# ChainSafe/Spectre

Hardware: NVIDIA H100
Metric: bn254_g1_msm_pairs_per_s (higher is better)
Workload: dtype u256 (8x32-bit Montgomery limbs, INT32 IMAD)

## Files before the change

### spectre_b200/csrc/common.cuh

```cuda
#pragma once
#include <cuda_runtime.h>
#include <stdint.h>
#include <stdio.h>
#include <string.h>
#include <initializer_list>
#include <map>
#include <mutex>
#include <string>
#include <vector>
#include "curve.cuh"
#include "../../include/spectre_b200.h"

namespace spb {


struct DevBuf {
  void* ptr = nullptr;
  size_t cap = 0;
};

struct NttTables {
  Fr omega;
  uint32_t k, h;
  Fr* tw_lo = nullptr;
  Fr* tw_hi = nullptr;
  Fr* tw_full = nullptr;
};

struct MsmLane {
  cudaStream_t stream = nullptr;
  cudaEvent_t ev[9] = {nullptr, nullptr, nullptr, nullptr, nullptr, nullptr, nullptr, nullptr, nullptr};
  void* pinned = nullptr;
  bool ready = false;
};
static const int kMaxMsmLanes = 3;

struct DeviceState {
  int device = 0;
  int sm_count = 0;
  size_t total_mem = 0;
  cudaStream_t stream = nullptr;
  cudaEvent_t ev0 = nullptr, ev1 = nullptr;
  cudaEvent_t dep_ev = nullptr;
  cudaEvent_t stage_ev[8] = {nullptr, nullptr, nullptr, nullptr, nullptr, nullptr, nullptr, nullptr};
  std::map<std::string, DevBuf> slots;
  MsmLane lanes[kMaxMsmLanes];
  std::vector<NttTables> ntt_tables;
  std::vector<NttTables> ntt_pre_tables;
  void* pinned = nullptr;
  size_t pinned_cap = 0;
  void* stage[2] = {nullptr, nullptr};
  cudaEvent_t stage_done[2] = {nullptr, nullptr};
};

}

struct spb_ctx {
  std::vector<spb::DeviceState> dev;
  std::mutex mu;
  std::string last_error;
  bool peer_access = false;
  uint64_t n_kernel_launches = 0;
  float last_kernel_ms = 0.f;
  uint64_t last_msm_adds = 0;
  bool shplonk_slots_busy = false;
  float msm_stage_ms[7] = {0, 0, 0, 0, 0, 0, 0};
};

struct spb_domain {
  uint32_t j, k, extended_k, quotient_poly_degree;
  spb::Fr omega, omega_inv, extended_omega, extended_omega_inv, g_coset, g_coset_inv, ifft_divisor, extended_ifft_divisor;
  uint32_t t_len;
  spb::Fr* d_t_evaluations;
  int device;
};

namespace spb {

int set_error(spb_ctx* ctx, int code, const char* fmt, ...);
void* slot(spb_ctx* ctx, DeviceState& d, const char* name, size_t bytes);

#define SPB_CUDA(ctx, call)                                                                      \
  do {                                                                                           \
    cudaError_t e_ = (call);                                                                     \
// ... 122 lines not shown
```

### spectre_b200/csrc/msm.cu

```cuda
#define SPB_MSM_KERNELS 1
#include "common.cuh"
#include "msm.cuh"
#include <cub/device/device_scan.cuh>
#include <string.h>

using namespace spb;

struct SrsShard {
  int dev_index = 0;
  size_t start = 0, count = 0;
  G1Affine* g = nullptr;
  G1Affine* g_lagrange = nullptr;
};
struct spb_srs {
  uint32_t k = 0;
  size_t n = 0;
  unsigned char g2[128] = {0}, s_g2[128] = {0};
  uint32_t table_c = 0;
  std::vector<SrsShard> shards;
};


namespace spb {

typedef MsmLane Lane;
static const size_t kLanePinnedBytes = 256 * 1024;
static int get_lane(spb_ctx* ctx, int dev_index, int lane_index, Lane** out) {
  Lane& l = ctx->dev[dev_index].lanes[lane_index];
  if (!l.ready) {
    SPB_CUDA(ctx, cudaStreamCreateWithFlags(&l.stream, cudaStreamNonBlocking));
    for (int i = 0; i < 9; i++) SPB_CUDA(ctx, cudaEventCreate(&l.ev[i]));
    SPB_CUDA(ctx, cudaMallocHost(&l.pinned, kLanePinnedBytes));
    l.ready = true;
  }
  *out = &l;
  return 0;
}

void msm_release_ctx(spb_ctx* ctx) {
  for (auto& d : ctx->dev) {
    cudaSetDevice(d.device);
    for (auto& l : d.lanes) {
      if (!l.ready) continue;
      cudaStreamSynchronize(l.stream);
      for (int i = 0; i < 9; i++) cudaEventDestroy(l.ev[i]);
      cudaFreeHost(l.pinned);
      cudaStreamDestroy(l.stream);
      l = Lane();
    }
  }
}

static void* lane_slot(spb_ctx* ctx, DeviceState& d, int lane, const char* name, size_t bytes) {
  char buf[64];
  snprintf(buf, sizeof buf, "%s#%d", name, lane);
  return slot(ctx, d, buf, bytes);
}

static uint32_t choose_chunk(const DeviceState& d, uint64_t est_entries) {
  const double wave = (double)d.sm_count * 512.0;
  if (est_entries >= kLongChunkMinEntries) return kLongChunk;
  double waves = (double)est_entries / 32.0 / wave;
  if (waves < 1.0) return 32;
  double w = waves < 1.5 ? 1.0 : (double)(uint64_t)(waves + 0.5);
  uint32_t L = (uint32_t)((double)est_entries / (w * wave)) + 1;
  if (L < 24) L = 24;
  if (L > 48) L = 48;
  return L;
}

static int msm_enqueue(spb_ctx* ctx, DeviceState& d, int lane, Lane& ln, const Fr* d_scalars, const G1Affine* d_bases, uint64_t n, MsmGeom g) {
  const uint64_t nb = (uint64_t)g.BW * g.B;
  const uint64_t cap = n * g.W;
  const uint32_t Lmin = g.L == kLongChunk ? kShortChunk : g.L;
  const uint64_t Tmax = (cap + Lmin - 1) / Lmin;
  if (cap >= 0x7fffffffull) return set_error(ctx, SPB_ERR_ARG, "msm: %llu entries exceed the 31-bit sort index", (unsigned long long)cap);
  uint32_t* counts = (uint32_t*)lane_slot(ctx, d, lane, "msm_counts", (nb + 1) * 4);
  uint32_t* offsets = (uint32_t*)lane_slot(ctx, d, lane, "msm_offsets", (nb + 1) * 4);
  MsmEntry* ent = (MsmEntry*)lane_slot(ctx, d, lane, "msm_entries", (cap + 1) * sizeof(MsmEntry));
  G1Xyzz* buckets = (G1Xyzz*)lane_slot(ctx, d, lane, "msm_buckets", nb * sizeof(G1Xyzz));
  uint32_t* head_key = (uint32_t*)lane_slot(ctx, d, lane, "msm_head_key", (Tmax + 1) * 4);
  uint32_t* tail_key = (uint32_t*)lane_slot(ctx, d, lane, "msm_tail_key", (Tmax + 1) * 4);
  G1Xyzz* head = (G1Xyzz*)lane_slot(ctx, d, lane, "msm_head", (Tmax + 1) * sizeof(G1Xyzz));
  G1Xyzz* tail = (G1Xyzz*)lane_slot(ctx, d, lane, "msm_tail", (Tmax + 1) * sizeof(G1Xyzz));
  uint32_t* giant = (uint32_t*)lane_slot(ctx, d, lane, "msm_giant", (Tmax + 2) * 4);
  const uint64_t max_huge = Tmax / kHugeChain + 1;
  uint32_t* huge = (uint32_t*)lane_slot(ctx, d, lane, "msm_huge", (2 * max_huge + 2) * 4);
  G1Xyzz* huge_part = (G1Xyzz*)lane_slot(ctx, d, lane, "msm_huge_part", max_huge * kHugeBlocks * sizeof(G1Xyzz));
  const MsmTail tl = msm_tail_shape(g.c);
  const uint32_t R = 1u << tl.r_log, C = 1u << tl.c_log, per = msm_tail_partials(tl);
  const uint32_t T1 = g.B >> tl.m_log;
  const uint64_t ngroups = (uint64_t)g.BW * T1;
  G1Xyzz* grp = (G1Xyzz*)lane_slot(ctx, d, lane, "msm_groups", 2 * ngroups * sizeof(G1Xyzz));
  G1Xyzz* seg_out = (G1Xyzz*)lane_slot(ctx, d, lane, "msm_rowcol", (uint64_t)g.BW * (2 * R + C) * sizeof(G1Xyzz));
  G1Xyzz* win_out = (G1Xyzz*)lane_slot(ctx, d, lane, "msm_partials", (uint64_t)g.BW * per * sizeof(G1Xyzz));
  size_t scan_bytes = 0;
  cub::DeviceScan::ExclusiveSum(nullptr, scan_bytes, counts, offsets, (int)(nb + 1), ln.stream);
  void* scan_tmp = lane_slot(ctx, d, lane, "msm_scan_tmp", scan_bytes ? scan_bytes : 16);
  if (!counts || !offsets || !ent || !buckets || !head_key || !tail_key || !head || !tail || !giant || !huge || !huge_part || !grp || !seg_out || !win_out || !scan_tmp)
    return SPB_ERR_OOM;
  if ((size_t)g.BW * per * sizeof(G1Xyzz) + 16 > kLanePinnedBytes) return set_error(ctx, SPB_ERR_STATE, "msm: %u window partials exceed the pinned staging area", g.BW * per);

  cudaStream_t st = ln.stream;
  SPB_CUDA(ctx, cudaMemsetAsync(giant, 0, 4, st));
  SPB_CUDA(ctx, cudaMemsetAsync(huge, 0, 4, st));
  const unsigned tb = 256;
  SPB_CUDA(ctx, cudaMemsetAsync(counts, 0, (nb + 1) * 4, st));
  cudaEventRecord(ln.ev[0], st);
  SPB_TRY(launch(ctx, st, nblk(n, tb), tb, 0, msm_count_kernel, n, d_scalars, g, counts));
  cudaEventRecord(ln.ev[1], st);
  SPB_CUDA(ctx, cub::DeviceScan::ExclusiveSum(scan_tmp, scan_bytes, counts, offsets, (int)(nb + 1), st));
  SPB_CUDA(ctx, cudaMemcpyAsync(counts, offsets, (nb + 1) * 4, cudaMemcpyDeviceToDevice, st));
  cudaEventRecord(ln.ev[2], st);
  SPB_TRY(launch(ctx, st, nblk(n, tb), tb, 0, msm_scatter_kernel, n, d_scalars, g, counts, ent));
  const uint32_t* total = offsets + nb;
  cudaEventRecord(ln.ev[3], st);
  SPB_TRY(launch(ctx, st, nblk(Tmax, 128), 128, 0, msm_accumulate_kernel, total, g, ent, d_bases, buckets, head_key, head, tail_key, tail));
  cudaEventRecord(ln.ev[4], st);
  SPB_TRY(launch(ctx, st, nblk(Tmax, 128), 128, 0, msm_stitch_kernel, total, g.L, 24, head_key, head, tail_key, tail, buckets, giant, giant + 1));
  SPB_TRY(launch(ctx, st, 256, 128, 0, msm_giant_kernel, total, g.L, giant, giant + 1, head_key, head, tail_key, tail, buckets, huge, huge + 2));
  SPB_TRY(launch(ctx, st, kHugeBlocks, 128, 0, msm_huge_kernel, huge, huge + 2, head, huge_part));
  SPB_TRY(launch(ctx, st, 64, 128, 0, msm_huge_finish_kernel, huge, huge + 2, kHugeBlocks, huge_part, tail_key, tail, buckets));
  cudaEventRecord(ln.ev[5], st);
  G1Xyzz *rows = seg_out, *cols = seg_out + (uint64_t)g.BW * R, *wrows = seg_out + (uint64_t)g.BW * (R + C);
  SPB_TRY(launch(ctx, st, nblk(ngroups, 128), 128, 0, msm_group_kernel, ngroups, tl.m_log, offsets, buckets, grp, grp + ngroups));
  cudaEventRecord(ln.ev[6], st);
  SPB_TRY(launch(ctx, st, g.BW * (2 * R + C), 64, 0, msm_rowcol_kernel, T1, tl, grp, grp + ngroups, rows, cols, wrows));
  SPB_TRY(launch(ctx, st, g.BW * (2 * tl.nbr + tl.nbc), 128, 0, msm_weighted_kernel, tl, rows, cols, wrows, win_out));
  cudaEventRecord(ln.ev[7], st);
  SPB_CUDA(ctx, cudaMemcpyAsync(ln.pinned, win_out, (size_t)g.BW * per * sizeof(G1Xyzz), cudaMemcpyDeviceToHost, st));
  SPB_CUDA(ctx, cudaMemcpyAsync((char*)ln.pinned + (size_t)g.BW * per * sizeof(G1Xyzz), total, 4, cudaMemcpyDeviceToHost, st));
  return 0;
}

static G1Xyzz msm_finish(Lane& ln, MsmGeom g, uint64_t* adds) {
  const MsmTail tl = msm_tail_shape(g.c);
  const uint32_t per = msm_tail_partials(tl);
  const G1Xyzz* P = (const G1Xyzz*)ln.pinned;
  uint32_t M; memcpy(&M, (const char*)ln.pinned + (size_t)g.BW * per * sizeof(G1Xyzz), 4);
  if (adds) *adds += (uint64_t)M + 2ull * g.BW * g.B;
  std::vector<G1Xyzz> S(g.BW);
  for (uint32_t w = 0; w < g.BW; w++) S[w] = msm_tail_finish(g, P + (size_t)w * per);
  return msm_combine_windows(S.data(), g.BW, g.c);
}

static void write_result(const G1Xyzz& r, spb_g1* out) {
  G1Affine a = xyzz_to_affine(r);
  G1Jac j = jac_from_affine(a);
  memcpy(out, &j, sizeof(G1Jac));
}

struct MsmPart {
  int dev_index;
  const Fr* d_scalars;
  const Fr* h_scalars;
  int peer_src_device;
  const G1Affine* d_bases;
  uint64_t n;
  MsmGeom g;
};

static int job_enqueue(spb_ctx* ctx, int lane, std::vector<MsmPart>& parts) {
  for (auto& p : parts) {
    if (!p.n) continue;
    DeviceState& d = ctx->dev[p.dev_index];
    SPB_CUDA(ctx, cudaSetDevice(d.device));
    Lane* ln; SPB_TRY(get_lane(ctx, p.dev_index, lane, &ln));
    p.g.L = choose_chunk(d, p.n * p.g.W);
    const Fr* ds = p.d_scalars;
    DeviceState& src = p.peer_src_device >= 0 ? ctx->dev[0] : d;
    if (&src != &d) SPB_CUDA(ctx, cudaSetDevice(src.device));
    SPB_CUDA(ctx, cudaEventRecord(src.dep_ev, src.stream));
    if (&src != &d) SPB_CUDA(ctx, cudaSetDevice(d.device));
    SPB_CUDA(ctx, cudaStreamWaitEvent(ln->stream, src.dep_ev, 0));
    SPB_CUDA(ctx, cudaEventRecord(ln->ev[8], ln->stream));
    if (p.h_scalars || p.peer_src_device >= 0) {
      Fr* buf = (Fr*)lane_slot(ctx, d, lane, "msm_scalars", p.n * sizeof(Fr));
      if (!buf) return SPB_ERR_OOM;
      if (p.h_scalars) SPB_CUDA(ctx, cudaMemcpyAsync(buf, p.h_scalars, p.n * sizeof(Fr), cudaMemcpyHostToDevice, ln->stream));
      else SPB_CUDA(ctx, cudaMemcpyPeerAsync(buf, d.device, p.d_scalars, p.peer_src_device, p.n * sizeof(Fr), ln->stream));
      ds = buf;
    }
    SPB_TRY(msm_enqueue(ctx, d, lane, *ln, ds, p.d_bases, p.n, p.g));
  }
  return 0;
}

static int job_collect(spb_ctx* ctx, int lane, const std::vector<MsmPart>& parts, spb_g1* out) {
  G1Xyzz acc = xyzz_identity();
  float worst = 0.f;
  for (auto& p : parts) {
    if (!p.n) continue;
    DeviceState& d = ctx->dev[p.dev_index];
    SPB_CUDA(ctx, cudaSetDevice(d.device));
    Lane* ln; SPB_TRY(get_lane(ctx, p.dev_index, lane, &ln));
    SPB_CUDA(ctx, cudaStreamSynchronize(ln->stream));
    float ms = 0.f;
    SPB_CUDA(ctx, cudaEventElapsedTime(&ms, ln->ev[8], ln->ev[7]));
    if (ms > worst) worst = ms;
    if (p.dev_index == 0) for (int e = 0; e < 7; e++) cudaEventElapsedTime(&ctx->msm_stage_ms[e], ln->ev[e], ln->ev[e + 1]);
    G1Xyzz r = msm_finish(*ln, p.g, &ctx->last_msm_adds);
    xyzz_add(acc, r);
  }
  ctx->last_kernel_ms = worst;
  write_result(acc, out);
  return 0;
}

static int g1_fixed_base_mul(spb_ctx* ctx, DeviceState& d, const Fr* scalars, size_t n, G1Affine* out) {
  return launch(ctx, d.stream, nblk(n, 128), 128, 0, g1_fixed_base_mul_kernel, scalars, n, out);
}

}

extern "C" {

uint64_t spb_last_msm_adds(spb_ctx* ctx) { return ctx ? ctx->last_msm_adds : 0; }
void spb_last_msm_stage_ms(spb_ctx* ctx, float out[7]) { if (!out) return; for (int i = 0; i < 7; i++) out[i] = ctx ? ctx->msm_stage_ms[i] : 0.f; }
void spb_msm_geometry(size_t n, int tables, uint32_t* c, uint32_t* windows) {
  MsmGeom g = msm_make_geometry(msm_choose_c(n ? n : 1, tables != 0), tables != 0, 0);
  if (c) *c = g.c;
  if (windows) *windows = g.W;
}

static spb_srs* srs_alloc(spb_ctx* ctx, uint32_t k) {
  spb_srs* s = new spb_srs();
  s->k = k; s->n = (size_t)1 << k;
  size_t D = ctx->dev.size();
  for (size_t i = 0; i < D; i++) {
    SrsShard sh; sh.dev_index = (int)i;
    sh.start = s->n * i / D; sh.count = s->n * (i + 1) / D - sh.start;
    s->shards.push_back(sh);
  }
  return s;
}

// ... 298 lines not shown
    if (!src) return set_error(ctx, SPB_ERR_STATE, "spb_srs_download: basis %d not resident", basis);
    DeviceState& d = ctx->dev[sh.dev_index];
    SPB_CUDA(ctx, cudaSetDevice(d.device));
    SPB_CUDA(ctx, cudaMemcpy((G1Affine*)out + (lo - start), src + (lo - sh.start), (hi - lo) * sizeof(G1Affine), cudaMemcpyDeviceToHost));
  }
  return 0;
}

int spb_msm_raw(spb_ctx* ctx, const spb_fr* scalars, const spb_g1_affine* bases, size_t n, spb_g1* out) {
  if (!ctx || !out || (n && (!scalars || !bases))) return SPB_ERR_ARG;
  std::lock_guard<std::mutex> lk(ctx->mu);
  ctx->last_msm_adds = 0;
  std::vector<MsmPart> parts;
  size_t D = ctx->dev.size();
  for (size_t i = 0; i < D; i++) {
    size_t lo = n * i / D, cnt = n * (i + 1) / D - lo;
    if (!cnt) continue;
    DeviceState& d = ctx->dev[i];
    SPB_CUDA(ctx, cudaSetDevice(d.device));
    Lane* ln; SPB_TRY(get_lane(ctx, (int)i, 0, &ln));
    G1Affine* db = (G1Affine*)slot(ctx, d, "msm_raw_bases", cnt * sizeof(G1Affine));
    if (!db) return SPB_ERR_OOM;
    SPB_CUDA(ctx, cudaMemcpyAsync(db, (const G1Affine*)bases + lo, cnt * sizeof(G1Affine), cudaMemcpyHostToDevice, ln->stream));
    MsmPart p; p.dev_index = (int)i; p.d_scalars = nullptr; p.h_scalars = (const Fr*)scalars + lo; p.peer_src_device = -1;
    p.d_bases = db; p.n = cnt; p.g = msm_choose_geometry(cnt);
    parts.push_back(p);
  }
  SPB_TRY(job_enqueue(ctx, 0, parts));
  return job_collect(ctx, 0, parts, out);
}

static int srs_parts(spb_ctx* ctx, const spb_srs* srs, int basis, const Fr* scalars, bool on_device, size_t n, std::vector<MsmPart>& parts) {
  if (n > srs->n) return set_error(ctx, SPB_ERR_ARG, "spb_msm: %zu scalars but the SRS has %zu points", n, srs->n);
  for (auto& sh : srs->shards) {
    if (sh.start >= n) continue;
    size_t cnt = (n - sh.start) < sh.count ? (n - sh.start) : sh.count;
    const G1Affine* b = basis == SPB_BASIS_G ? sh.g : sh.g_lagrange;
    if (!b) return set_error(ctx, SPB_ERR_STATE, "spb_msm: basis %d not resident", basis);
    MsmPart p; p.dev_index = sh.dev_index; p.d_bases = b; p.n = cnt; p.h_scalars = nullptr; p.d_scalars = nullptr; p.peer_src_device = -1;
    if (!on_device) p.h_scalars = scalars + sh.start;
    else { p.d_scalars = scalars + sh.start; if (sh.dev_index != 0) p.peer_src_device = ctx->dev[0].device; }
    p.g = srs->table_c ? msm_make_geometry(srs->table_c, true, (uint32_t)sh.count) : msm_choose_geometry(cnt);
    parts.push_back(p);
  }
  return 0;
}

static int msm_batch_common(spb_ctx* ctx, const spb_srs* srs, int basis, const spb_fr* const* scalars, bool on_device, size_t n, size_t count, spb_g1* out) {
  if (!ctx || !srs || !out || (count && !scalars)) return SPB_ERR_ARG;
  std::lock_guard<std::mutex> lk(ctx->mu);
  ctx->last_msm_adds = 0;
  const MsmGeom lg = srs->table_c ? msm_make_geometry(srs->table_c, true, 0) : msm_choose_geometry(n ? n : 1);
  const uint64_t ents = (uint64_t)n * lg.W;
  const uint64_t lane_bytes = ents * sizeof(MsmEntry) + 2 * (ents / kShortChunk + 1) * (sizeof(G1Xyzz) + 4) + (uint64_t)lg.BW * lg.B * sizeof(G1Xyzz);
  const uint64_t fit = ctx->dev[0].total_mem / 10 / (lane_bytes ? lane_bytes : 1);
  const size_t NL = std::max<size_t>(1, std::min<size_t>((size_t)kMaxMsmLanes, (size_t)fit));
  std::vector<MsmPart> jobs[kMaxMsmLanes];
  for (size_t i = 0; i < count; i++) {
    int lane = (int)(i % NL);
    if (i >= NL) SPB_TRY(job_collect(ctx, lane, jobs[lane], &out[i - NL]));
    if (n && !scalars[i]) return SPB_ERR_ARG;
    jobs[lane].clear();
    SPB_TRY(srs_parts(ctx, srs, basis, (const Fr*)scalars[i], on_device, n, jobs[lane]));
    SPB_TRY(job_enqueue(ctx, lane, jobs[lane]));
  }
  for (size_t i = count >= NL ? count - NL : 0; i < count; i++) SPB_TRY(job_collect(ctx, (int)(i % NL), jobs[i % NL], &out[i]));
  return 0;
}

int spb_msm(spb_ctx* ctx, const spb_srs* srs, int basis, const spb_fr* scalars, size_t n, spb_g1* out) {
  const spb_fr* one[1] = {scalars};
  if (n && !scalars) return SPB_ERR_ARG;
  return msm_batch_common(ctx, srs, basis, one, false, n, 1, out);
}
int spb_msm_dev(spb_ctx* ctx, const spb_srs* srs, int basis, const spb_fr* d_scalars, size_t n, spb_g1* out) {
  const spb_fr* one[1] = {d_scalars};
  if (n && !d_scalars) return SPB_ERR_ARG;
  return msm_batch_common(ctx, srs, basis, one, true, n, 1, out);
}
int spb_msm_batch(spb_ctx* ctx, const spb_srs* srs, int basis, const spb_fr* const* scalars, size_t n, size_t count, spb_g1* out) {
  return msm_batch_common(ctx, srs, basis, scalars, false, n, count, out);
}
int spb_msm_batch_dev(spb_ctx* ctx, const spb_srs* srs, int basis, const spb_fr* const* d_scalars, size_t n, size_t count, spb_g1* out) {
  return msm_batch_common(ctx, srs, basis, d_scalars, true, n, count, out);
}

int spb_srs_precompute(spb_ctx* ctx, spb_srs* srs) {
  if (!ctx || !srs) return SPB_ERR_ARG;
  std::lock_guard<std::mutex> lk(ctx->mu);
  if (srs->table_c) return 0;
  size_t per_dev = srs->shards.empty() ? srs->n : srs->shards[0].count;
  uint32_t c = msm_choose_c(per_dev ? per_dev : 1, true);
  uint32_t W = (255 + c - 1) / c;
  for (auto& sh : srs->shards) {
    if (!sh.count) continue;
    SPB_CUDA(ctx, cudaSetDevice(ctx->dev[sh.dev_index].device));
    size_t free_b = 0, total_b = 0;
    SPB_CUDA(ctx, cudaMemGetInfo(&free_b, &total_b));
    const size_t bases = (sh.g ? 1 : 0) + (sh.g_lagrange ? 1 : 0);
    if ((size_t)W * sh.count * sizeof(G1Affine) * bases > total_b / 4) return 0;
  }
  for (auto& sh : srs->shards) {
    if (!sh.count) continue;
    DeviceState& d = ctx->dev[sh.dev_index];
    SPB_CUDA(ctx, cudaSetDevice(d.device));
    if ((uint64_t)W * sh.count >= 0x7fffffffull) return set_error(ctx, SPB_ERR_ARG, "spb_srs_precompute: table index exceeds 31 bits");
    for (int which = 0; which < 2; which++) {
// ... 26 lines not shown
```

### spectre_b200/csrc/msm.cuh

```cuda
#pragma once
#include <stdlib.h>
#include "curve.cuh"

namespace spb {

struct MsmGeom {
  uint32_t c;
  uint32_t W;
  uint32_t B;
  uint32_t L;
  uint32_t BW;
  uint32_t precomp;
  uint32_t tab_stride;
};

struct alignas(8) MsmEntry { uint32_t key, val; };

static const uint32_t kLongChunk = 96, kShortChunk = 32;
#ifndef SPB_LONG_CHUNK_MIN_ENTRIES
#define SPB_LONG_CHUNK_MIN_ENTRIES (1ull << 23)
#endif
static const uint64_t kLongChunkMinEntries = SPB_LONG_CHUNK_MIN_ENTRIES;
SPB_HD uint32_t msm_effective_chunk(uint32_t L, uint64_t M) { return (L == kLongChunk && M < kLongChunkMinEntries) ? kShortChunk : L; }

static const uint32_t kNoKey = 0xffffffffu;

#if defined(__CUDA_ARCH__)
SPB_D uint32_t spb_atomic_inc(uint32_t* p) { return atomicAdd(p, 1u); }
#else
inline uint32_t spb_atomic_inc(uint32_t* p) { uint32_t v = *p; *p = v + 1; return v; }
#endif

struct DigitIter {
  uint32_t limbs[8];
  uint32_t c, carry, w;
  SPB_HD void init(const Fr& canonical, uint32_t c_) {
    for (int i = 0; i < 8; i++) limbs[i] = canonical.l[i];
    c = c_; carry = 0; w = 0;
  }
  SPB_HD int32_t next() {
    uint32_t bit = w * c, word = bit >> 5, sh = bit & 31;
    uint64_t v = 0;
    if (word < 8) {
      v = limbs[word];
      if (word + 1 < 8) v |= (uint64_t)limbs[word + 1] << 32;
      v >>= sh;
    }
    uint32_t raw = (uint32_t)(v & ((1u << c) - 1)) + carry;
    w++;
    if (raw > (1u << (c - 1))) { carry = 1; return (int32_t)raw - (int32_t)(1u << c); }
    carry = 0;
    return (int32_t)raw;
  }
};

SPB_HD void msm_count_thread(uint64_t tid, uint64_t n, const Fr* scalars, MsmGeom g, uint32_t* counts) {
  if (tid >= n) return;
  Fr s = fp_from_mont(scalars[tid]);
  if (fp_is_zero(s)) return;
  DigitIter it; it.init(s, g.c);
  for (uint32_t w = 0; w < g.W; w++) {
    int32_t d = it.next();
    if (d == 0) continue;
    uint32_t mag = d < 0 ? (uint32_t)(-d) : (uint32_t)d;
    spb_atomic_inc(&counts[(g.precomp ? 0u : w * g.B) + mag - 1]);
  }
}

SPB_HD void msm_scatter_thread(uint64_t tid, uint64_t n, const Fr* scalars, MsmGeom g, uint32_t* cursor, MsmEntry* ent) {
  if (tid >= n) return;
  Fr s = fp_from_mont(scalars[tid]);
  if (fp_is_zero(s)) return;
  DigitIter it; it.init(s, g.c);
  for (uint32_t w = 0; w < g.W; w++) {
    int32_t d = it.next();
    if (d == 0) continue;
    uint32_t mag = d < 0 ? (uint32_t)(-d) : (uint32_t)d;
    uint32_t key = (g.precomp ? 0u : w * g.B) + mag - 1;
    uint32_t pos = spb_atomic_inc(&cursor[key]);
    MsmEntry e; e.key = key; e.val = ((uint32_t)tid + (g.precomp ? w * g.tab_stride : 0u)) | (d < 0 ? 0x80000000u : 0u);
    ent[pos] = e;
  }
}

SPB_HD G1Affine msm_load_point(const G1Affine* bases, uint32_t val) {
#if defined(__CUDA_ARCH__)
  const uint4* q = reinterpret_cast<const uint4*>(bases + (val & 0x7fffffffu));
  uint4 a = __ldg(q), b = __ldg(q + 1), c = __ldg(q + 2), d = __ldg(q + 3);
  G1Affine p;
  p.x.l[0] = a.x; p.x.l[1] = a.y; p.x.l[2] = a.z; p.x.l[3] = a.w; p.x.l[4] = b.x; p.x.l[5] = b.y; p.x.l[6] = b.z; p.x.l[7] = b.w;
  p.y.l[0] = c.x; p.y.l[1] = c.y; p.y.l[2] = c.z; p.y.l[3] = c.w; p.y.l[4] = d.x; p.y.l[5] = d.y; p.y.l[6] = d.z; p.y.l[7] = d.w;
#else
  G1Affine p = bases[val & 0x7fffffffu];
#endif
  if (val & 0x80000000u) p.y = fp_neg(p.y);
  return p;
}

SPB_HD MsmEntry msm_load_entry(const MsmEntry* p) {
#if defined(__CUDA_ARCH__)
  uint2 v = __ldg(reinterpret_cast<const uint2*>(p));
  MsmEntry e; e.key = v.x; e.val = v.y; return e;
#else
  return *p;
#endif
}

// ... 83 lines not shown
  uint32_t R = 1u << t.r_log, C = 1u << t.c_log, per = msm_tail_partials(t);
  const uint64_t T = (uint64_t)g.B >> t.m_log;
  G1Xyzz* s1 = (G1Xyzz*)malloc(sizeof(G1Xyzz) * T * g.BW);
  G1Xyzz* w1 = (G1Xyzz*)malloc(sizeof(G1Xyzz) * T * g.BW);
  for (uint64_t tid = 0; tid < T * g.BW; tid++) msm_group_thread(tid, T * g.BW, t.m_log, offsets, buckets, s1, w1);
  for (uint32_t w = 0; w < g.BW; w++) {
    const G1Xyzz* X = s1 + (uint64_t)w * T;
    const G1Xyzz* V = w1 + (uint64_t)w * T;
    G1Xyzz* out = partials + (uint64_t)w * per;
    for (uint32_t i = 0; i < per; i++) out[i] = xyzz_identity();
    for (uint32_t r = 0; r < R; r++) {
      G1Xyzz row = xyzz_identity(), wrow = xyzz_identity();
      for (uint32_t c = 0; c < C; c++) { xyzz_add(row, X[(uint64_t)r * C + c]); xyzz_add(wrow, V[(uint64_t)r * C + c]); }
      G1Xyzz wr = xyzz_mul_u32(row, r % 128);
      xyzz_add(out[r / 128], wr);
      xyzz_add(out[t.nbr + r / 128], row);
      xyzz_add(out[2 * t.nbr + 2 * t.nbc + r / 128], wrow);
    }
    for (uint32_t c = 0; c < C; c++) {
      G1Xyzz col = xyzz_identity();
      for (uint32_t r = 0; r < R; r++) xyzz_add(col, X[(uint64_t)r * C + c]);
      G1Xyzz wc = xyzz_mul_u32(col, c % 128);
      xyzz_add(out[2 * t.nbr + c / 128], wc);
      xyzz_add(out[2 * t.nbr + t.nbc + c / 128], col);
    }
  }
  free(s1); free(w1);
}
inline G1Xyzz msm_tail_finish(const MsmGeom& g, const G1Xyzz* part) {
  MsmTail t = msm_tail_shape(g.c);
  auto fold = [](const G1Xyzz* X, const G1Xyzz* Y, uint32_t nb, G1Xyzz* plain) {
    G1Xyzz sx = xyzz_identity(), run = xyzz_identity(), wsum = xyzz_identity();
    for (int j = (int)nb - 1; j >= 0; j--) {
      xyzz_add(sx, X[j]);
      if (j >= 1) { xyzz_add(run, Y[j]); xyzz_add(wsum, run); }
    }
    if (plain) { *plain = run; xyzz_add(*plain, Y[0]); }
    for (int i = 0; i < 7; i++) wsum = xyzz_dbl(wsum);
    xyzz_add(sx, wsum);
    return sx;
  };
  G1Xyzz S;
  G1Xyzz A = fold(part, part + t.nbr, t.nbr, &S);
  G1Xyzz D = fold(part + 2 * t.nbr, part + 2 * t.nbr + t.nbc, t.nbc, nullptr);
  for (uint32_t i = 0; i < t.c_log; i++) A = xyzz_dbl(A);
  xyzz_add(A, D);
  for (uint32_t i = 0; i < t.m_log; i++) A = xyzz_dbl(A);
  xyzz_add(A, S);
  for (uint32_t j = 0; j < t.nbr; j++) xyzz_add(A, part[2 * t.nbr + 2 * t.nbc + j]);
  return A;
}

#if defined(__CUDACC__) && defined(SPB_MSM_KERNELS)
__device__ __forceinline__ unsigned msm_warp_peers(uint32_t key, uint32_t lane) {
  const uint32_t next = __shfl_down_sync(0xffffffffu, key, 1);
  const bool dup = lane < 31u && next == key && key != kNoKey;
  if (__any_sync(0xffffffffu, dup)) return __match_any_sync(0xffffffffu, key);
  return 1u << lane;
}
__global__ void msm_count_kernel(uint64_t n, const Fr* scalars, MsmGeom g, uint32_t* counts) {
  const uint64_t tid = blockIdx.x * (uint64_t)blockDim.x + threadIdx.x;
  const uint32_t lane = threadIdx.x & 31u;
  bool live = tid < n;
  Fr s = live ? fp_from_mont(scalars[tid]) : fp_zero<FrParams>();
  live = live && !fp_is_zero(s);
  DigitIter it; it.init(s, g.c);
  for (uint32_t w = 0; w < g.W; w++) {
    int32_t d = it.next();
    const bool act = live && d != 0;
    const uint32_t mag = d < 0 ? (uint32_t)(-d) : (uint32_t)d;
    const uint32_t key = (g.precomp ? 0u : w * g.B) + mag - 1;
    const unsigned peers = msm_warp_peers(act ? key : kNoKey, lane);
    if (act && lane == (uint32_t)(__ffs(peers) - 1)) atomicAdd(&counts[key], (uint32_t)__popc(peers));
  }
}
__global__ void msm_scatter_kernel(uint64_t n, const Fr* scalars, MsmGeom g, uint32_t* cursor, MsmEntry* ent) {
  const uint64_t tid = blockIdx.x * (uint64_t)blockDim.x + threadIdx.x;
  const uint32_t lane = threadIdx.x & 31u;
  bool live = tid < n;
  Fr s = live ? fp_from_mont(scalars[tid]) : fp_zero<FrParams>();
  live = live && !fp_is_zero(s);
  DigitIter it; it.init(s, g.c);
  for (uint32_t w = 0; w < g.W; w++) {
    int32_t d = it.next();
    const bool act = live && d != 0;
    const uint32_t mag = d < 0 ? (uint32_t)(-d) : (uint32_t)d;
    const uint32_t key = (g.precomp ? 0u : w * g.B) + mag - 1;
    const unsigned peers = msm_warp_peers(act ? key : kNoKey, lane);
    const uint32_t leader = (uint32_t)(__ffs(peers) - 1);
    uint32_t base = 0;
    if (act && lane == leader) base = atomicAdd(&cursor[key], (uint32_t)__popc(peers));
    base = __shfl_sync(0xffffffffu, base, leader);
    if (act) {
      const uint32_t pos = base + (uint32_t)__popc(peers & ((1u << lane) - 1u));
      MsmEntry e; e.key = key; e.val = ((uint32_t)tid + (g.precomp ? w * g.tab_stride : 0u)) | (d < 0 ? 0x80000000u : 0u);
      ent[pos] = e;
    }
  }
}
#ifndef SPB_ACC_MINBLOCKS
#define SPB_ACC_MINBLOCKS 1
#endif
__global__ void __launch_bounds__(128, SPB_ACC_MINBLOCKS) msm_accumulate_kernel(const uint32_t* total, MsmGeom g, const MsmEntry* ent,
                                                             const G1Affine* bases, G1Xyzz* buckets, uint32_t* head_key, G1Xyzz* head,
                                                             uint32_t* tail_key, G1Xyzz* tail) {
  msm_accumulate_thread(blockIdx.x * (uint64_t)blockDim.x + threadIdx.x, *total, g, ent, bases, buckets, head_key, head, tail_key, tail);
}
__global__ void __launch_bounds__(128) msm_stitch_kernel(const uint32_t* total, uint32_t L, uint32_t cap, const uint32_t* head_key, const G1Xyzz* head,
                                                         const uint32_t* tail_key, const G1Xyzz* tail, G1Xyzz* buckets, uint32_t* giant_count, uint32_t* giant_list) {
  L = msm_effective_chunk(L, *total);
  uint64_t T = ((uint64_t)*total + L - 1) / L;
  msm_stitch_thread(blockIdx.x * (uint64_t)blockDim.x + threadIdx.x, T, cap, head_key, head, tail_key, tail, buckets, giant_count, giant_list);
}

template <int NT>
__device__ void block_sum_xyzz(G1Xyzz& v, G1Xyzz* sh) {
  const int tid = threadIdx.x;
  for (int stride = NT / 2; stride >= 1; stride >>= 1) {
    if (tid >= stride && tid < 2 * stride) sh[tid - stride] = v;
    __syncthreads();
    if (tid < stride) xyzz_add(v, sh[tid]);
    __syncthreads();
  }
}

template <int NT>
__device__ void block_sum2_xyzz(G1Xyzz& a, G1Xyzz& b, G1Xyzz* sh ) {
  const int tid = threadIdx.x;
  for (int stride = NT / 2; stride >= 1; stride >>= 1) {
    if (tid >= stride && tid < 2 * stride) { sh[2 * (tid - stride)] = a; sh[2 * (tid - stride) + 1] = b; }
    __syncthreads();
    if (tid < stride) { xyzz_add(a, sh[2 * tid]); xyzz_add(b, sh[2 * tid + 1]); }
    __syncthreads();
  }
}

static const uint32_t kHugeChain = 4096;
static const uint32_t kHugeBlocks = 1056;
__global__ void __launch_bounds__(128) msm_giant_kernel(const uint32_t* total, uint32_t L, const uint32_t* giant_count, const uint32_t* giant_list,
                                                        const uint32_t* head_key, const G1Xyzz* head, const uint32_t* tail_key, const G1Xyzz* tail,
                                                        G1Xyzz* buckets, uint32_t* huge_count, uint32_t* huge_list ) {
  __shared__ G1Xyzz sh[64];
  __shared__ uint64_t s_end;
  L = msm_effective_chunk(L, *total);
  const uint64_t T = ((uint64_t)*total + L - 1) / L;
  const uint32_t count = *giant_count;
  for (uint32_t gi = blockIdx.x; gi < count; gi += gridDim.x) {
    uint64_t t0 = giant_list[gi];
    uint32_t key = tail_key[t0];
    if (threadIdx.x == 0) {
      uint64_t lo = t0 + 1, hi = T;
// ... 207 lines not shown
```

### spectre_b200/halo2.py

```python
import ctypes
import os

import numpy as np

_HERE = os.path.dirname(os.path.abspath(__file__))
LIB_PATH = os.environ.get("SPB_LIB_PATH") or os.path.join(_HERE, "libspectre_b200.so")

R_MOD = 0x30644e72e131a029b85045b68181585d2833e84879b9709143e1f593f0000001
P_MOD = 0x30644e72e131a029b85045b68181585d97816a916871ca8d3c208c16d87cfd47
MONT_RADIX = 1 << 256
FQ_MONT_INV = pow(MONT_RADIX, -1, P_MOD)


def g1_on_curve(x, y):
    return x < P_MOD and y < P_MOD and (y * y - x * x * x - 3) % P_MOD == 0


BASIS_G = 0
BASIS_G_LAGRANGE = 1

ERR_DATA = -6
SERDE_FORMATS = {"RawBytes": 1, "RawBytesUnchecked": 2}


# ... 57 lines not shown

    def __init__(self, devices=None):
        self.lib = load_library()
        devices = list(devices) if devices is not None else [0]
        ids = (ctypes.c_int * len(devices))(*devices)
        self.ctx = self.lib.spb_init(ids, len(devices))
        if not self.ctx:
            raise BackendError("spb_init failed: no usable CUDA device (the library has no CPU fallback)")
        self.ctx = ctypes.c_void_p(self.ctx)
        self.devices = devices

    def close(self):
        if getattr(self, "ctx", None):
            self.lib.spb_shutdown(self.ctx)
            self.ctx = None

    def __del__(self):
        try:
            self.close()
        except Exception:
            pass

    def check(self, rc, what):
        if rc != 0:
            raise BackendError("%s failed (%d): %s" % (what, rc, self.lib.spb_last_error(self.ctx).decode()))

    def release_workspace(self):
        self.check(self.lib.spb_release_workspace(self.ctx), "spb_release_workspace")

    def stream(self, dev_index=0):
        self.lib.spb_stream.restype = ctypes.c_void_p
        self.lib.spb_stream.argtypes = [ctypes.c_void_p, ctypes.c_int]
        s = self.lib.spb_stream(self.ctx, dev_index)
        if not s:
            raise BackendError("spb_stream: no stream for device index %d" % dev_index)
        return int(s)

    @property
    def kernel_launches(self):
        return int(self.lib.spb_kernel_launches(self.ctx))

    @property
    def last_device_ms(self):
        return float(self.lib.spb_last_device_ms(self.ctx))

    @property
    def last_msm_adds(self):
        return int(self.lib.spb_last_msm_adds(self.ctx))

    @property
    def last_msm_stage_ms(self):
        out = (ctypes.c_float * 7)()
        self.lib.spb_last_msm_stage_ms(self.ctx, out)
        return dict(zip(("count", "scan", "scatter", "accumulate", "stitch", "groups", "rowcol_weighted"), [float(v) for v in out]))

    def msm_geometry(self, n, tables=False):
        c = ctypes.c_uint32(); w = ctypes.c_uint32()
        self.lib.spb_msm_geometry(ctypes.c_size_t(n), ctypes.c_int(1 if tables else 0), ctypes.byref(c), ctypes.byref(w))
        return c.value, w.value

    def best_fft(self, a, omega, log_n):
        a = _fr_array(a).copy()
        assert a.shape[0] == 1 << log_n, "best_fft: a.len() != 1 << log_n"
        omega = _fr_array(omega, 1)
        self.check(self.lib.spb_ntt(self.ctx, _p(a), ctypes.c_uint32(log_n), _p(omega)), "spb_ntt")
        return a

    def best_fft_dev(self, d_ptr, omega, log_n):
        omega = _fr_array(omega, 1)
        self.check(self.lib.spb_ntt_dev(self.ctx, _p(d_ptr), ctypes.c_uint32(log_n), _p(omega)), "spb_ntt_dev")

    def best_multiexp(self, coeffs, bases):
        coeffs = _fr_array(coeffs)
        bases = np.ascontiguousarray(bases, dtype=np.uint64).reshape(-1, 8)
        assert coeffs.shape[0] == bases.shape[0], "best_multiexp: coeffs.len() != bases.len()"
        out = np.empty(12, dtype=np.uint64)
        self.check(self.lib.spb_msm_raw(self.ctx, _p(coeffs), _p(bases), ctypes.c_size_t(coeffs.shape[0]), _p(out)), "spb_msm_raw")
        return out

    def pairing(self, ps, qs):
        ps, qs = _pair_arrays(ps, qs)
        out = np.empty((12, 4), dtype=np.uint64)
        self.check(self.lib.spb_pairing(self.ctx, _p(ps), _p(qs), ctypes.c_size_t(ps.shape[0]), _p(out)), "spb_pairing")
        return out

    def pairing_check_batch(self, ps, qs, m):
        ps, qs = _pair_arrays(ps, qs)
        if m <= 0 or ps.shape[0] % m:
            raise ValueError("pairing_check_batch: %d pairs do not split into checks of m = %d" % (ps.shape[0], m))
        n_checks = ps.shape[0] // m
        ok = np.zeros(max(n_checks, 1), dtype=np.int32)
        self.check(self.lib.spb_pairing_check_batch(self.ctx, _p(ps), _p(qs), ctypes.c_size_t(m), ctypes.c_size_t(n_checks), _p(ok)), "spb_pairing_check_batch")
        return [bool(v) for v in ok[:n_checks]]

    def batch_invert(self, a):
        a = _fr_array(a).copy()
        self.check(self.lib.spb_batch_invert(self.ctx, _p(a), ctypes.c_size_t(a.shape[0])), "spb_batch_invert")
        return a

    def eval_polynomial(self, poly, point):
        poly = _fr_array(poly); point = _fr_array(point, 1)
        out = np.empty(4, dtype=np.uint64)
        self.check(self.lib.spb_eval_polynomial(self.ctx, _p(poly), ctypes.c_size_t(poly.shape[0]), _p(point), _p(out)), "spb_eval_polynomial")
        return out

    def kate_division(self, a, b):
        a = _fr_array(a); b = _fr_array(b, 1)
# ... 504 lines not shown
```

Before: 289.9 million.

## Replace count/scan/scatter bucket binning with digit emission plus CUB radix sort

The two-pass bucket binning (count kernel with warp-aggregated atomics, exclusive scan, then a scatter kernel) is replaced by one digits kernel that writes (key, point) entries compactly with block-level atomics. A CUB radix sort over the used key bits then orders them, and a binary-search kernel derives the bucket offsets. This removes the second pass over the scalars and the contended per-bucket atomics. In exchange it needs a double-buffered entry array and a host sync to read back the entry count before sorting, which splits enqueue into two phases.

```diff
diff --git a/spectre_b200/csrc/common.cuh b/spectre_b200/csrc/common.cuh
--- a/spectre_b200/csrc/common.cuh
+++ b/spectre_b200/csrc/common.cuh
@@ -29,7 +29,7 @@
 
 struct MsmLane {
   cudaStream_t stream = nullptr;
-  cudaEvent_t ev[9] = {nullptr, nullptr, nullptr, nullptr, nullptr, nullptr, nullptr, nullptr, nullptr};
+  cudaEvent_t ev[10] = {nullptr, nullptr, nullptr, nullptr, nullptr, nullptr, nullptr, nullptr, nullptr, nullptr};
   void* pinned = nullptr;
   bool ready = false;
 };
diff --git a/spectre_b200/csrc/msm.cu b/spectre_b200/csrc/msm.cu
--- a/spectre_b200/csrc/msm.cu
+++ b/spectre_b200/csrc/msm.cu
@@ -1,7 +1,7 @@
 #define SPB_MSM_KERNELS 1
 #include "common.cuh"
 #include "msm.cuh"
-#include <cub/device/device_scan.cuh>
+#include <cub/device/device_radix_sort.cuh>
 #include <string.h>
 
 using namespace spb;
@@ -29,7 +29,7 @@
   Lane& l = ctx->dev[dev_index].lanes[lane_index];
   if (!l.ready) {
     SPB_CUDA(ctx, cudaStreamCreateWithFlags(&l.stream, cudaStreamNonBlocking));
-    for (int i = 0; i < 9; i++) SPB_CUDA(ctx, cudaEventCreate(&l.ev[i]));
+    for (int i = 0; i < 10; i++) SPB_CUDA(ctx, cudaEventCreate(&l.ev[i]));
     SPB_CUDA(ctx, cudaMallocHost(&l.pinned, kLanePinnedBytes));
     l.ready = true;
   }
@@ -43,7 +43,7 @@
     for (auto& l : d.lanes) {
       if (!l.ready) continue;
       cudaStreamSynchronize(l.stream);
-      for (int i = 0; i < 9; i++) cudaEventDestroy(l.ev[i]);
+      for (int i = 0; i < 10; i++) cudaEventDestroy(l.ev[i]);
       cudaFreeHost(l.pinned);
       cudaStreamDestroy(l.stream);
       l = Lane();
@@ -69,15 +69,46 @@
   return L;
 }
 
-static int msm_enqueue(spb_ctx* ctx, DeviceState& d, int lane, Lane& ln, const Fr* d_scalars, const G1Affine* d_bases, uint64_t n, MsmGeom g) {
+struct MsmWork {
+  uint32_t* total;
+  MsmEntry* ent[2];
+  void* sort_tmp; size_t sort_bytes;
+};
+static int msm_work(spb_ctx* ctx, DeviceState& d, int lane, Lane& ln, uint64_t n, MsmGeom g, MsmWork& w) {
+  const uint64_t cap = n * g.W;
+  if (cap >= 0x7fffffffull) return set_error(ctx, SPB_ERR_ARG, "msm: %llu entries exceed the 31-bit sort index", (unsigned long long)cap);
+  w.total = (uint32_t*)lane_slot(ctx, d, lane, "msm_total", 16);
+  w.ent[0] = (MsmEntry*)lane_slot(ctx, d, lane, "msm_entries", (cap + 1) * sizeof(MsmEntry));
+  w.ent[1] = (MsmEntry*)lane_slot(ctx, d, lane, "msm_entries_alt", (cap + 1) * sizeof(MsmEntry));
+  cub::DoubleBuffer<uint64_t> keys((uint64_t*)w.ent[0], (uint64_t*)w.ent[1]);
+  w.sort_bytes = 0;
+  SPB_CUDA(ctx, cub::DeviceRadixSort::SortKeys(nullptr, w.sort_bytes, keys, (int)cap, 0, msm_key_bits(g), ln.stream));
+  w.sort_tmp = lane_slot(ctx, d, lane, "msm_sort_tmp", w.sort_bytes ? w.sort_bytes : 16);
+  if (!w.total || !w.ent[0] || !w.ent[1] || !w.sort_tmp) return SPB_ERR_OOM;
+  return 0;
+}
+
+static int msm_enqueue_digits(spb_ctx* ctx, DeviceState& d, int lane, Lane& ln, const Fr* d_scalars, uint64_t n, MsmGeom g) {
+  MsmWork w; SPB_TRY(msm_work(ctx, d, lane, ln, n, g, w));
+  const uint32_t per = msm_tail_partials(msm_tail_shape(g.c));
+  if ((size_t)g.BW * per * sizeof(G1Xyzz) + 16 > kLanePinnedBytes) return set_error(ctx, SPB_ERR_STATE, "msm: %u window partials exceed the pinned staging area", g.BW * per);
+  cudaStream_t st = ln.stream;
+  SPB_CUDA(ctx, cudaMemsetAsync(w.total, 0, 4, st));
+  cudaEventRecord(ln.ev[0], st);
+  SPB_TRY(launch(ctx, st, nblk(n, kDigitsThreads), kDigitsThreads, 0, msm_digits_kernel, n, d_scalars, g, w.total, w.ent[0]));
+  cudaEventRecord(ln.ev[1], st);
+  SPB_CUDA(ctx, cudaMemcpyAsync((char*)ln.pinned + (size_t)g.BW * per * sizeof(G1Xyzz), w.total, 4, cudaMemcpyDeviceToHost, st));
+  SPB_CUDA(ctx, cudaEventRecord(ln.ev[9], st));
+  return 0;
+}
+
+static int msm_enqueue_rest(spb_ctx* ctx, DeviceState& d, int lane, Lane& ln, const G1Affine* d_bases, uint64_t n, MsmGeom g) {
+  MsmWork w; SPB_TRY(msm_work(ctx, d, lane, ln, n, g, w));
   const uint64_t nb = (uint64_t)g.BW * g.B;
   const uint64_t cap = n * g.W;
   const uint32_t Lmin = g.L == kLongChunk ? kShortChunk : g.L;
   const uint64_t Tmax = (cap + Lmin - 1) / Lmin;
-  if (cap >= 0x7fffffffull) return set_error(ctx, SPB_ERR_ARG, "msm: %llu entries exceed the 31-bit sort index", (unsigned long long)cap);
-  uint32_t* counts = (uint32_t*)lane_slot(ctx, d, lane, "msm_counts", (nb + 1) * 4);
   uint32_t* offsets = (uint32_t*)lane_slot(ctx, d, lane, "msm_offsets", (nb + 1) * 4);
-  MsmEntry* ent = (MsmEntry*)lane_slot(ctx, d, lane, "msm_entries", (cap + 1) * sizeof(MsmEntry));
   G1Xyzz* buckets = (G1Xyzz*)lane_slot(ctx, d, lane, "msm_buckets", nb * sizeof(G1Xyzz));
   uint32_t* head_key = (uint32_t*)lane_slot(ctx, d, lane, "msm_head_key", (Tmax + 1) * 4);
   uint32_t* tail_key = (uint32_t*)lane_slot(ctx, d, lane, "msm_tail_key", (Tmax + 1) * 4);
@@ -94,26 +125,20 @@
   G1Xyzz* grp = (G1Xyzz*)lane_slot(ctx, d, lane, "msm_groups", 2 * ngroups * sizeof(G1Xyzz));
   G1Xyzz* seg_out = (G1Xyzz*)lane_slot(ctx, d, lane, "msm_rowcol", (uint64_t)g.BW * (2 * R + C) * sizeof(G1Xyzz));
   G1Xyzz* win_out = (G1Xyzz*)lane_slot(ctx, d, lane, "msm_partials", (uint64_t)g.BW * per * sizeof(G1Xyzz));
-  size_t scan_bytes = 0;
-  cub::DeviceScan::ExclusiveSum(nullptr, scan_bytes, counts, offsets, (int)(nb + 1), ln.stream);
-  void* scan_tmp = lane_slot(ctx, d, lane, "msm_scan_tmp", scan_bytes ? scan_bytes : 16);
-  if (!counts || !offsets || !ent || !buckets || !head_key || !tail_key || !head || !tail || !giant || !huge || !huge_part || !grp || !seg_out || !win_out || !scan_tmp)
+  if (!offsets || !buckets || !head_key || !tail_key || !head || !tail || !giant || !huge || !huge_part || !grp || !seg_out || !win_out)
     return SPB_ERR_OOM;
-  if ((size_t)g.BW * per * sizeof(G1Xyzz) + 16 > kLanePinnedBytes) return set_error(ctx, SPB_ERR_STATE, "msm: %u window partials exceed the pinned staging area", g.BW * per);
-
+
+  SPB_CUDA(ctx, cudaEventSynchronize(ln.ev[9]));
+  uint32_t M; memcpy(&M, (const char*)ln.pinned + (size_t)g.BW * per * sizeof(G1Xyzz), 4);
   cudaStream_t st = ln.stream;
   SPB_CUDA(ctx, cudaMemsetAsync(giant, 0, 4, st));
   SPB_CUDA(ctx, cudaMemsetAsync(huge, 0, 4, st));
-  const unsigned tb = 256;
-  SPB_CUDA(ctx, cudaMemsetAsync(counts, 0, (nb + 1) * 4, st));
-  cudaEventRecord(ln.ev[0], st);
-  SPB_TRY(launch(ctx, st, nblk(n, tb), tb, 0, msm_count_kernel, n, d_scalars, g, counts));
-  cudaEventRecord(ln.ev[1], st);
-  SPB_CUDA(ctx, cub::DeviceScan::ExclusiveSum(scan_tmp, scan_bytes, counts, offsets, (int)(nb + 1), st));
-  SPB_CUDA(ctx, cudaMemcpyAsync(counts, offsets, (nb + 1) * 4, cudaMemcpyDeviceToDevice, st));
+  cub::DoubleBuffer<uint64_t> keys((uint64_t*)w.ent[0], (uint64_t*)w.ent[1]);
+  SPB_CUDA(ctx, cub::DeviceRadixSort::SortKeys(w.sort_tmp, w.sort_bytes, keys, (int)M, 0, msm_key_bits(g), st));
+  const MsmEntry* ent = (const MsmEntry*)keys.Current();
+  const uint32_t* total = w.total;
   cudaEventRecord(ln.ev[2], st);
-  SPB_TRY(launch(ctx, st, nblk(n, tb), tb, 0, msm_scatter_kernel, n, d_scalars, g, counts, ent));
-  const uint32_t* total = offsets + nb;
+  SPB_TRY(launch(ctx, st, nblk(nb + 1, 256), 256, 0, msm_offsets_kernel, total, nb, ent, offsets));
   cudaEventRecord(ln.ev[3], st);
   SPB_TRY(launch(ctx, st, nblk(Tmax, 128), 128, 0, msm_accumulate_kernel, total, g, ent, d_bases, buckets, head_key, head, tail_key, tail));
   cudaEventRecord(ln.ev[4], st);
@@ -129,7 +154,6 @@
   SPB_TRY(launch(ctx, st, g.BW * (2 * tl.nbr + tl.nbc), 128, 0, msm_weighted_kernel, tl, rows, cols, wrows, win_out));
   cudaEventRecord(ln.ev[7], st);
   SPB_CUDA(ctx, cudaMemcpyAsync(ln.pinned, win_out, (size_t)g.BW * per * sizeof(G1Xyzz), cudaMemcpyDeviceToHost, st));
-  SPB_CUDA(ctx, cudaMemcpyAsync((char*)ln.pinned + (size_t)g.BW * per * sizeof(G1Xyzz), total, 4, cudaMemcpyDeviceToHost, st));
   return 0;
 }
 
@@ -181,7 +205,14 @@
       else SPB_CUDA(ctx, cudaMemcpyPeerAsync(buf, d.device, p.d_scalars, p.peer_src_device, p.n * sizeof(Fr), ln->stream));
       ds = buf;
     }
-    SPB_TRY(msm_enqueue(ctx, d, lane, *ln, ds, p.d_bases, p.n, p.g));
+    SPB_TRY(msm_enqueue_digits(ctx, d, lane, *ln, ds, p.n, p.g));
+  }
+  for (auto& p : parts) {
+    if (!p.n) continue;
+    DeviceState& d = ctx->dev[p.dev_index];
+    SPB_CUDA(ctx, cudaSetDevice(d.device));
+    Lane* ln; SPB_TRY(get_lane(ctx, p.dev_index, lane, &ln));
+    SPB_TRY(msm_enqueue_rest(ctx, d, lane, *ln, p.d_bases, p.n, p.g));
   }
   return 0;
 }
@@ -586,7 +617,7 @@
   ctx->last_msm_adds = 0;
   const MsmGeom lg = srs->table_c ? msm_make_geometry(srs->table_c, true, 0) : msm_choose_geometry(n ? n : 1);
   const uint64_t ents = (uint64_t)n * lg.W;
-  const uint64_t lane_bytes = ents * sizeof(MsmEntry) + 2 * (ents / kShortChunk + 1) * (sizeof(G1Xyzz) + 4) + (uint64_t)lg.BW * lg.B * sizeof(G1Xyzz);
+  const uint64_t lane_bytes = 2 * ents * sizeof(MsmEntry) + 2 * (ents / kShortChunk + 1) * (sizeof(G1Xyzz) + 4) + (uint64_t)lg.BW * lg.B * sizeof(G1Xyzz);
   const uint64_t fit = ctx->dev[0].total_mem / 10 / (lane_bytes ? lane_bytes : 1);
   const size_t NL = std::max<size_t>(1, std::min<size_t>((size_t)kMaxMsmLanes, (size_t)fit));
   std::vector<MsmPart> jobs[kMaxMsmLanes];
diff --git a/spectre_b200/csrc/msm.cuh b/spectre_b200/csrc/msm.cuh
--- a/spectre_b200/csrc/msm.cuh
+++ b/spectre_b200/csrc/msm.cuh
@@ -53,6 +53,48 @@
     return (int32_t)raw;
   }
 };
+
+SPB_HD MsmEntry msm_make_entry(uint64_t tid, uint32_t w, int32_t d, const MsmGeom& g) {
+  const uint32_t mag = d < 0 ? (uint32_t)(-d) : (uint32_t)d;
+  MsmEntry e;
+  e.key = (g.precomp ? 0u : w * g.B) + mag - 1;
+  e.val = ((uint32_t)tid + (g.precomp ? w * g.tab_stride : 0u)) | (d < 0 ? 0x80000000u : 0u);
+  return e;
+}
+SPB_HD uint32_t msm_digit_count(const Fr& s, const MsmGeom& g) {
+  DigitIter it; it.init(s, g.c);
+  uint32_t k = 0;
+  for (uint32_t w = 0; w < g.W; w++) k += it.next() != 0;
+  return k;
+}
+SPB_HD void msm_digits_thread(uint64_t tid, uint64_t n, const Fr* scalars, MsmGeom g, uint32_t* total, MsmEntry* ent) {
+  if (tid >= n) return;
+  Fr s = fp_from_mont(scalars[tid]);
+  if (fp_is_zero(s)) return;
+  uint32_t pos = *total;
+  *total = pos + msm_digit_count(s, g);
+  DigitIter it; it.init(s, g.c);
+  for (uint32_t w = 0; w < g.W; w++) {
+    int32_t d = it.next();
+    if (d != 0) ent[pos++] = msm_make_entry(tid, w, d, g);
+  }
+}
+
+inline int msm_key_bits(const MsmGeom& g) {
+  int bits = 0;
+  for (uint64_t k = (uint64_t)g.BW * g.B - 1; k; k >>= 1) bits++;
+  return bits;
+}
+
+SPB_HD void msm_offsets_thread(uint64_t k, uint64_t nb, uint64_t M, const MsmEntry* sorted, uint32_t* offsets) {
+  if (k > nb) return;
+  uint64_t lo = 0, hi = M;
+  while (lo < hi) {
+    const uint64_t mid = (lo + hi) >> 1;
+    if (sorted[mid].key < k) lo = mid + 1; else hi = mid;
+  }
+  offsets[k] = (uint32_t)lo;
+}
 
 SPB_HD void msm_count_thread(uint64_t tid, uint64_t n, const Fr* scalars, MsmGeom g, uint32_t* counts) {
   if (tid >= n) return;
@@ -242,51 +284,37 @@
 }
 
 #if defined(__CUDACC__) && defined(SPB_MSM_KERNELS)
-__device__ __forceinline__ unsigned msm_warp_peers(uint32_t key, uint32_t lane) {
-  const uint32_t next = __shfl_down_sync(0xffffffffu, key, 1);
-  const bool dup = lane < 31u && next == key && key != kNoKey;
-  if (__any_sync(0xffffffffu, dup)) return __match_any_sync(0xffffffffu, key);
-  return 1u << lane;
-}
-__global__ void msm_count_kernel(uint64_t n, const Fr* scalars, MsmGeom g, uint32_t* counts) {
+static const unsigned kDigitsThreads = 256;
+__global__ void __launch_bounds__(kDigitsThreads) msm_digits_kernel(uint64_t n, const Fr* scalars, MsmGeom g, uint32_t* total, MsmEntry* ent) {
+  __shared__ uint32_t s_warp[kDigitsThreads / 32];
+  __shared__ uint32_t s_base;
   const uint64_t tid = blockIdx.x * (uint64_t)blockDim.x + threadIdx.x;
-  const uint32_t lane = threadIdx.x & 31u;
+  const uint32_t lane = threadIdx.x & 31u, warp = threadIdx.x >> 5;
   bool live = tid < n;
   Fr s = live ? fp_from_mont(scalars[tid]) : fp_zero<FrParams>();
   live = live && !fp_is_zero(s);
+  uint32_t wsum = live ? msm_digit_count(s, g) : 0u;
+  for (int o = 16; o; o >>= 1) wsum += __shfl_xor_sync(0xffffffffu, wsum, o);
+  if (lane == 0) s_warp[warp] = wsum;
+  __syncthreads();
+  if (threadIdx.x == 0) {
+    uint32_t run = 0;
+    for (unsigned i = 0; i < kDigitsThreads / 32; i++) { const uint32_t v = s_warp[i]; s_warp[i] = run; run += v; }
+    s_base = run ? atomicAdd(total, run) : 0u;
+  }
+  __syncthreads();
+  uint32_t pos = s_base + s_warp[warp];
   DigitIter it; it.init(s, g.c);
   for (uint32_t w = 0; w < g.W; w++) {
-    int32_t d = it.next();
+    const int32_t d = it.next();
     const bool act = live && d != 0;
-    const uint32_t mag = d < 0 ? (uint32_t)(-d) : (uint32_t)d;
-    const uint32_t key = (g.precomp ? 0u : w * g.B) + mag - 1;
-    const unsigned peers = msm_warp_peers(act ? key : kNoKey, lane);
-    if (act && lane == (uint32_t)(__ffs(peers) - 1)) atomicAdd(&counts[key], (uint32_t)__popc(peers));
-  }
-}
-__global__ void msm_scatter_kernel(uint64_t n, const Fr* scalars, MsmGeom g, uint32_t* cursor, MsmEntry* ent) {
-  const uint64_t tid = blockIdx.x * (uint64_t)blockDim.x + threadIdx.x;
-  const uint32_t lane = threadIdx.x & 31u;
-  bool live = tid < n;
-  Fr s = live ? fp_from_mont(scalars[tid]) : fp_zero<FrParams>();
-  live = live && !fp_is_zero(s);
-  DigitIter it; it.init(s, g.c);
-  for (uint32_t w = 0; w < g.W; w++) {
-    int32_t d = it.next();
-    const bool act = live && d != 0;
-    const uint32_t mag = d < 0 ? (uint32_t)(-d) : (uint32_t)d;
-    const uint32_t key = (g.precomp ? 0u : w * g.B) + mag - 1;
-    const unsigned peers = msm_warp_peers(act ? key : kNoKey, lane);
-    const uint32_t leader = (uint32_t)(__ffs(peers) - 1);
-    uint32_t base = 0;
-    if (act && lane == leader) base = atomicAdd(&cursor[key], (uint32_t)__popc(peers));
-    base = __shfl_sync(0xffffffffu, base, leader);
-    if (act) {
-      const uint32_t pos = base + (uint32_t)__popc(peers & ((1u << lane) - 1u));
-      MsmEntry e; e.key = key; e.val = ((uint32_t)tid + (g.precomp ? w * g.tab_stride : 0u)) | (d < 0 ? 0x80000000u : 0u);
-      ent[pos] = e;
-    }
-  }
+    const unsigned m = __ballot_sync(0xffffffffu, act);
+    if (act) ent[pos + (uint32_t)__popc(m & ((1u << lane) - 1u))] = msm_make_entry(tid, w, d, g);
+    pos += (uint32_t)__popc(m);
+  }
+}
+__global__ void __launch_bounds__(256) msm_offsets_kernel(const uint32_t* total, uint64_t nb, const MsmEntry* sorted, uint32_t* offsets) {
+  msm_offsets_thread(blockIdx.x * (uint64_t)blockDim.x + threadIdx.x, nb, *total, sorted, offsets);
 }
 #ifndef SPB_ACC_MINBLOCKS
 #define SPB_ACC_MINBLOCKS 1
diff --git a/spectre_b200/halo2.py b/spectre_b200/halo2.py
--- a/spectre_b200/halo2.py
+++ b/spectre_b200/halo2.py
@@ -133,7 +133,7 @@
     def last_msm_stage_ms(self):
         out = (ctypes.c_float * 7)()
         self.lib.spb_last_msm_stage_ms(self.ctx, out)
-        return dict(zip(("count", "scan", "scatter", "accumulate", "stitch", "groups", "rowcol_weighted"), [float(v) for v in out]))
+        return dict(zip(("digits", "sort", "offsets", "accumulate", "stitch", "groups", "rowcol_weighted"), [float(v) for v in out]))
 
     def msm_geometry(self, n, tables=False):
         c = ctypes.c_uint32(); w = ctypes.c_uint32()
```

New measurement: 328.1 million (median of 6 runs). 1.13x the previous value.
